# submission2019/cnn-quantization

Measured on NVIDIA H100. Metric: resnet50_w4a4_images_per_s, higher is better.
Workload: dtype f32

## Files before the change

cnn-quantization_b200/csrc/fq_bulk.cuh:

```cuda
#pragma once
#include <cuda_runtime.h>
#include <stdint.h>

#include "fq_device.cuh"

namespace fqb {

constexpr int kConsumers = kThreads;
constexpr int kBulkThreads = kConsumers + 32;
constexpr int kConsumerWarps = kConsumers / 32;
#ifndef FQB_STAGE_VEC
#define FQB_STAGE_VEC 4
#endif
#ifndef FQB_STAGES
#define FQB_STAGES 6
#endif
#ifndef FQB_BULK_CTAS
#define FQB_BULK_CTAS 1
#endif
constexpr int kBulkCtasPerSm = FQB_BULK_CTAS;
constexpr int kStageVec = FQB_STAGE_VEC;
constexpr int kStages = FQB_STAGES;
constexpr unsigned kStageBytes = kStageVec * kConsumers * 16u;
#ifndef FQB_BULK_SPLIT
#define FQB_BULK_SPLIT 1
#endif
constexpr unsigned kBulkSplit = FQB_BULK_SPLIT;

__device__ __forceinline__ void consumer_sync() { cta_sync(); }

__device__ __forceinline__ unsigned smem_u32(const void* p) { return static_cast<unsigned>(__cvta_generic_to_shared(p)); }
__device__ __forceinline__ void mbar_init(unsigned bar, unsigned count) {
  asm volatile("mbarrier.init.shared::cta.b64 [%0], %1;" ::"r"(bar), "r"(count) : "memory");
}
__device__ __forceinline__ void mbar_fence_init() { asm volatile("fence.mbarrier_init.release.cluster;" ::: "memory"); }
__device__ __forceinline__ void mbar_arrive(unsigned bar) {
  asm volatile("{ .reg .b64 st; mbarrier.arrive.shared::cta.b64 st, [%0]; }" ::"r"(bar) : "memory");
}
__device__ __forceinline__ void mbar_arrive_expect_tx(unsigned bar, unsigned bytes) {
  asm volatile("{ .reg .b64 st; mbarrier.arrive.expect_tx.shared::cta.b64 st, [%0], %1; }" ::"r"(bar), "r"(bytes) : "memory");
}
__device__ __forceinline__ bool mbar_try_wait(unsigned bar, unsigned parity) {
  unsigned ok;
  asm volatile(
      "{ .reg .pred p; mbarrier.try_wait.parity.shared::cta.b64 p, [%1], %2; selp.u32 %0, 1, 0, p; }"
      : "=r"(ok)
      : "r"(bar), "r"(parity)
      : "memory");
  return ok != 0;
}
__device__ __forceinline__ void mbar_wait(unsigned bar, unsigned parity) {
  while (!mbar_try_wait(bar, parity)) {
  }
}
__device__ __forceinline__ void bulk_load_one(unsigned dst_smem, const void* src, unsigned bytes, unsigned bar) {
  asm volatile("cp.async.bulk.shared::cluster.global.mbarrier::complete_tx::bytes [%0], [%1], %2, [%3];" ::"r"(dst_smem),
               "l"(src), "r"(bytes), "r"(bar)
               : "memory");
}
__device__ __forceinline__ void bulk_load(unsigned dst_smem, const void* src, unsigned bytes, unsigned bar) {
  if (kBulkSplit == 1u) {
    bulk_load_one(dst_smem, src, bytes, bar);
    return;
  }
  constexpr unsigned piece = kStageBytes / kBulkSplit;
  for (unsigned off = 0; off < bytes; off += piece)
    bulk_load_one(dst_smem + off, static_cast<const unsigned char*>(src) + off, min(piece, bytes - off), bar);
}

struct FlatGeo {
  unsigned total_v;
  unsigned stride;
  unsigned stage_v;
  unsigned n_stages;
  unsigned unit_stages;
  unsigned units;
  unsigned channels;
  unsigned cv;
};

struct StageMeta {
  unsigned start;
  unsigned count;
  unsigned tag;
  unsigned pad;
};

struct BulkRing {
  alignas(8) unsigned long long full[kStages];
  alignas(8) unsigned long long empty[kStages];
  StageMeta meta[kStages];
  unsigned nstages;
};

struct RingPos {
  unsigned slot, parity, n;
  __device__ __forceinline__ void init(unsigned nstages = kStages) {
    slot = 0;
    parity = 0;
    n = nstages;
  }
  __device__ __forceinline__ void next() {
    if (++slot == n) {
      slot = 0;
      parity ^= 1u;
    }
  }
};

__device__ __forceinline__ void ring_init(BulkRing& r, unsigned nstages = kStages) {
  if (threadIdx.x == 0) {
    r.nstages = nstages;
#pragma unroll
    for (int s = 0; s < kStages; ++s) {
      mbar_init(smem_u32(&r.full[s]), 1u);
      mbar_init(smem_u32(&r.empty[s]), kConsumerWarps);
    }
    mbar_fence_init();
  }
  __syncthreads();
}

struct TicketPlan {
  unsigned nstatic;
  unsigned first, step;
  unsigned dyn_base;
};

constexpr unsigned kPairOffset = kStageBytes / 2u;

__device__ __forceinline__ FlatGeo half_geo(const FlatGeo& g) {
  FlatGeo h = g;
  h.stage_v = (kStageVec / 2u) * g.stride;
  h.n_stages = (g.total_v + h.stage_v - 1u) / h.stage_v;
  h.unit_stages = 2u * g.unit_stages;
  return h;
}

template <bool REV, bool PAIR = false>
__device__ __forceinline__ void produce_phase(const FlatGeo& g, const float4* src, unsigned* counter, const TicketPlan tp,
                                              BulkRing& r, unsigned char* stage_base, RingPos& pos,
                                              const float4* src2 = nullptr) {
  const unsigned total = g.units;
  unsigned k = 0;
  auto fetch = [&]() -> unsigned {
    unsigned long long t;
    if (k < tp.nstatic)
      t = tp.first + static_cast<unsigned long long>(k) * tp.step;
    else
      t = static_cast<unsigned long long>(tp.dyn_base) + atomicAdd(counter, 1u);
    ++k;
    return t < total ? static_cast<unsigned>(t) : 0xffffffffu;
  };
  unsigned cur = fetch();
  unsigned nxt = (cur != 0xffffffffu) ? fetch() : 0xffffffffu;
  while (cur != 0xffffffffu) {
    const unsigned nxt2 = (nxt != 0xffffffffu) ? fetch() : 0xffffffffu;
    const unsigned u = REV ? total - 1u - cur : cur;
    const unsigned g0 = u * g.unit_stages;
    const unsigned g1 = min(g0 + g.unit_stages, g.n_stages);
    for (unsigned i = g0; i < g1; ++i) {
      const unsigned st = REV ? g1 - 1u - (i - g0) : i;
      const unsigned start = st * g.stage_v;
      const unsigned count = min(g.stage_v, g.total_v - start);
      mbar_wait(smem_u32(&r.empty[pos.slot]), pos.parity ^ 1u);
      r.meta[pos.slot].start = start;
      r.meta[pos.slot].count = count;
      r.meta[pos.slot].tag = 0u;
      const unsigned bar = smem_u32(&r.full[pos.slot]);
      mbar_arrive_expect_tx(bar, PAIR ? count * 32u : count * 16u);
      bulk_load(smem_u32(stage_base + pos.slot * kStageBytes), src + start, count * 16u, bar);
      if (PAIR) bulk_load(smem_u32(stage_base + pos.slot * kStageBytes + kPairOffset), src2 + start, count * 16u, bar);
      pos.next();
    }
    cur = nxt;
    nxt = nxt2;
  }
  mbar_wait(smem_u32(&r.empty[pos.slot]), pos.parity ^ 1u);
  r.meta[pos.slot].start = 0u;
  r.meta[pos.slot].count = 0u;
  mbar_arrive(smem_u32(&r.full[pos.slot]));
  pos.next();
}

struct RowsGeo {
  unsigned rows, row_v;
  unsigned stages_per_row;
  unsigned units_per_row;
};

__device__ __forceinline__ RowsGeo half_rows(const FlatGeo& h, const RowsGeo& rg) {
  RowsGeo r = rg;
  r.stages_per_row = (rg.row_v + h.stage_v - 1u) / h.stage_v;
  r.units_per_row = (r.stages_per_row + h.unit_stages - 1u) / h.unit_stages;
  return r;
}

template <bool REV, bool PAIR = false>
__device__ __forceinline__ void produce_rows_phase(const FlatGeo& g, const RowsGeo& rg, const float4* src, unsigned* counter,
                                                   const TicketPlan tp, BulkRing& r, unsigned char* stage_base, RingPos& pos,
                                                   const float4* src2 = nullptr) {
  const unsigned total = g.units;
  unsigned k = 0;
  auto fetch = [&]() -> unsigned {
    unsigned long long t;
    if (k < tp.nstatic)
      t = tp.first + static_cast<unsigned long long>(k) * tp.step;
    else
      t = static_cast<unsigned long long>(tp.dyn_base) + atomicAdd(counter, 1u);
    ++k;
    return t < total ? static_cast<unsigned>(t) : 0xffffffffu;
  };
  unsigned cur = fetch();
  unsigned nxt = (cur != 0xffffffffu) ? fetch() : 0xffffffffu;
  while (cur != 0xffffffffu) {
    const unsigned nxt2 = (nxt != 0xffffffffu) ? fetch() : 0xffffffffu;
    const unsigned u = REV ? total - 1u - cur : cur;
    const unsigned row = u / rg.units_per_row;
    const unsigned part = u - row * rg.units_per_row;
    const unsigned s0 = part * g.unit_stages;
    const unsigned s1 = min(s0 + g.unit_stages, rg.stages_per_row);
    for (unsigned i = s0; i < s1; ++i) {
      const unsigned st = REV ? s1 - 1u - (i - s0) : i;
      const unsigned off = st * g.stage_v;
      const unsigned start = row * rg.row_v + off;
      const unsigned count = min(g.stage_v, rg.row_v - off);
      mbar_wait(smem_u32(&r.empty[pos.slot]), pos.parity ^ 1u);
      r.meta[pos.slot].start = start;
      r.meta[pos.slot].count = count;
      r.meta[pos.slot].tag = row | (i + 1u == s1 ? 0x80000000u : 0u);
      const unsigned bar = smem_u32(&r.full[pos.slot]);
      mbar_arrive_expect_tx(bar, PAIR ? count * 32u : count * 16u);
      bulk_load(smem_u32(stage_base + pos.slot * kStageBytes), src + start, count * 16u, bar);
      if (PAIR) bulk_load(smem_u32(stage_base + pos.slot * kStageBytes + kPairOffset), src2 + start, count * 16u, bar);
      pos.next();
    }
    cur = nxt;
    nxt = nxt2;
  }
  mbar_wait(smem_u32(&r.empty[pos.slot]), pos.parity ^ 1u);
  r.meta[pos.slot].start = 0u;
  r.meta[pos.slot].count = 0u;
  r.meta[pos.slot].tag = 0u;
  mbar_arrive(smem_u32(&r.full[pos.slot]));
  pos.next();
}

struct PoolGeo {
  unsigned h, w;
  unsigned wt;
  unsigned tiles_per_row;
  unsigned row_pairs;
  unsigned tiles;
  unsigned unit_tiles, units;
  unsigned ow;
  unsigned kind;
};

constexpr unsigned kPoolTop = 1u, kPoolLeft = 2u;

__device__ __forceinline__ void produce_pool3_phase(const FlatGeo& g, const PoolGeo& pg, const float4* src, unsigned* counter,
                                                    const TicketPlan tp, BulkRing& r, unsigned char* stage_base, RingPos& pos) {
  const unsigned total = pg.units;
  unsigned k = 0;
  auto fetch = [&]() -> unsigned {
    unsigned long long t;
    if (k < tp.nstatic)
      t = tp.first + static_cast<unsigned long long>(k) * tp.step;
    else
      t = static_cast<unsigned long long>(tp.dyn_base) + atomicAdd(counter, 1u);
    ++k;
    return t < total ? static_cast<unsigned>(t) : 0xffffffffu;
  };
  const unsigned row_v = pg.w * g.cv;
  const unsigned region_v = (2u * pg.wt + 1u) * g.cv;
  const unsigned per_img = pg.row_pairs * pg.tiles_per_row;
  unsigned cur = fetch();
  unsigned nxt = (cur != 0xffffffffu) ? fetch() : 0xffffffffu;
  while (cur != 0xffffffffu) {
    const unsigned nxt2 = (nxt != 0xffffffffu) ? fetch() : 0xffffffffu;
    const unsigned t0 = cur * pg.unit_tiles;
    const unsigned t1 = min(t0 + pg.unit_tiles, pg.tiles);
    for (unsigned tile = t0; tile < t1; ++tile) {
      const unsigned n = tile / per_img;
      const unsigned rem = tile - n * per_img;
      const unsigned oh = rem / pg.tiles_per_row;
      const unsigned wi = rem - oh * pg.tiles_per_row;
      const bool top = oh > 0u, left = wi > 0u;
      const unsigned skip = left ? 0u : g.cv;
      const unsigned count = region_v - skip;
      const unsigned mid = (n * pg.h + 2u * oh) * row_v + (2u * wi * pg.wt) * g.cv - (left ? g.cv : 0u);
      const unsigned o = ((n * pg.row_pairs + oh) * pg.ow + wi * pg.wt) * g.cv;
      mbar_wait(smem_u32(&r.empty[pos.slot]), pos.parity ^ 1u);
      r.meta[pos.slot].start = o;
      r.meta[pos.slot].count = count;
      r.meta[pos.slot].tag = (top ? kPoolTop : 0u) | (left ? kPoolLeft : 0u);
      const unsigned bar = smem_u32(&r.full[pos.slot]);
      mbar_arrive_expect_tx(bar, count * 16u * (top ? 3u : 2u));
      const unsigned dst = smem_u32(stage_base + pos.slot * kStageBytes) + skip * 16u;
      if (top) bulk_load(dst, src + mid - row_v, count * 16u, bar);
      bulk_load(dst + region_v * 16u, src + mid, count * 16u, bar);
      bulk_load(dst + 2u * region_v * 16u, src + mid + row_v, count * 16u, bar);
      pos.next();
    }
    cur = nxt;
    nxt = nxt2;
  }
  mbar_wait(smem_u32(&r.empty[pos.slot]), pos.parity ^ 1u);
  r.meta[pos.slot].start = 0u;
  r.meta[pos.slot].count = 0u;
  r.meta[pos.slot].tag = 0u;
  mbar_arrive(smem_u32(&r.full[pos.slot]));
  pos.next();
}

template <typename Acc>
__device__ __forceinline__ void consume_pool3_phase(const FlatGeo& g, const PoolGeo& pg, BulkRing& r, const unsigned char* stage_base,
                                                    RingPos& pos, Acc& acc) {
  const unsigned t = threadIdx.x;
  const bool lane0 = (t & 31u) == 0u;
  const bool mine = t < pg.wt * g.cv;
  const unsigned j = t / g.cv, col = t - j * g.cv;
  const unsigned region = (2u * pg.wt + 1u) * g.cv * 16u;
  const unsigned my = smem_u32(stage_base) + ((2u * j) * g.cv + col) * 16u;
  const unsigned nxt = g.cv * 16u;
  for (;;) {
    mbar_wait(smem_u32(&r.full[pos.slot]), pos.parity);
    const StageMeta m = r.meta[pos.slot];
    if (m.count != 0u && mine) {
      const unsigned addr = my + pos.slot * kStageBytes;
      const bool first = (j != 0u) || (m.tag & kPoolLeft);
      acc.pool_begin();
#pragma unroll
      for (int dy = 0; dy < 3; ++dy) {
        if (dy == 0 && !(m.tag & kPoolTop)) continue;
        const unsigned row = addr + dy * region;
        float4 v;
        if (first) {
          lds_vec(row, v);
          acc.pool_tap(v);
        }
        lds_vec(row + nxt, v);
        acc.pool_tap(v);
        lds_vec(row + 2u * nxt, v);
        acc.pool_tap(v);
      }
      acc.pool_end(m.start + t);
    }
    __syncwarp();
    if (lane0) mbar_arrive(smem_u32(&r.empty[pos.slot]));
    pos.next();
    if (m.count == 0u) break;
  }
}

__device__ __forceinline__ void produce_pool_phase(const FlatGeo& g, const PoolGeo& pg, const float4* src, unsigned* counter,
                                                   const TicketPlan tp, BulkRing& r, unsigned char* stage_base, RingPos& pos) {
  const unsigned total = pg.units;
  unsigned k = 0;
  auto fetch = [&]() -> unsigned {
    unsigned long long t;
    if (k < tp.nstatic)
      t = tp.first + static_cast<unsigned long long>(k) * tp.step;
    else
      t = static_cast<unsigned long long>(tp.dyn_base) + atomicAdd(counter, 1u);
    ++k;
    return t < total ? static_cast<unsigned>(t) : 0xffffffffu;
  };
  const unsigned row_v = pg.w * g.cv;
  const unsigned count = pg.wt * g.cv;
  const unsigned per_img = pg.row_pairs * pg.tiles_per_row;
  unsigned cur = fetch();
  unsigned nxt = (cur != 0xffffffffu) ? fetch() : 0xffffffffu;
  while (cur != 0xffffffffu) {
    const unsigned nxt2 = (nxt != 0xffffffffu) ? fetch() : 0xffffffffu;
    const unsigned t0 = cur * pg.unit_tiles;
    const unsigned t1 = min(t0 + pg.unit_tiles, pg.tiles);
    for (unsigned tile = t0; tile < t1; ++tile) {
      const unsigned n = tile / per_img;
      const unsigned rem = tile - n * per_img;
      const unsigned hp = rem / pg.tiles_per_row;
      const unsigned wi = rem - hp * pg.tiles_per_row;
      const unsigned a = (n * pg.h + 2u * hp) * row_v + wi * count;
      const unsigned o = ((n * pg.row_pairs + hp) * pg.ow + wi * (pg.wt / 2u)) * g.cv;
      mbar_wait(smem_u32(&r.empty[pos.slot]), pos.parity ^ 1u);
      r.meta[pos.slot].start = o;
      r.meta[pos.slot].count = count;
      r.meta[pos.slot].tag = 0u;
      const unsigned bar = smem_u32(&r.full[pos.slot]);
      mbar_arrive_expect_tx(bar, count * 32u);
      bulk_load(smem_u32(stage_base + pos.slot * kStageBytes), src + a, count * 16u, bar);
      bulk_load(smem_u32(stage_base + pos.slot * kStageBytes + kPairOffset), src + a + row_v, count * 16u, bar);
      pos.next();
    }
    cur = nxt;
    nxt = nxt2;
  }
  mbar_wait(smem_u32(&r.empty[pos.slot]), pos.parity ^ 1u);
  r.meta[pos.slot].start = 0u;
  r.meta[pos.slot].count = 0u;
  r.meta[pos.slot].tag = 0u;
  mbar_arrive(smem_u32(&r.full[pos.slot]));
  pos.next();
}

template <typename Acc>
__device__ __forceinline__ void consume_pool_phase(const FlatGeo& g, const PoolGeo& pg, BulkRing& r, const unsigned char* stage_base,
                                                   RingPos& pos, Acc& acc) {
  const unsigned t = threadIdx.x;
  const bool lane0 = (t & 31u) == 0u;
  const bool mine = t < (pg.wt / 2u) * g.cv;
  const unsigned j = t / g.cv, col = t - j * g.cv;
  const unsigned my = smem_u32(stage_base) + ((2u * j) * g.cv + col) * 16u;
  const unsigned nxt = g.cv * 16u;
  for (;;) {
    mbar_wait(smem_u32(&r.full[pos.slot]), pos.parity);
    const StageMeta m = r.meta[pos.slot];
    if (m.count != 0u && mine) {
      const unsigned addr = my + pos.slot * kStageBytes;
      float4 a0, a1, b0, b1;
      lds_vec(addr, a0);
      lds_vec(addr + nxt, a1);
      lds_vec(addr + kPairOffset, b0);
      lds_vec(addr + kPairOffset + nxt, b1);
      acc.pooled(a0, a1, b0, b1, m.start + t);
    }
    __syncwarp();
    if (lane0) mbar_arrive(smem_u32(&r.empty[pos.slot]));
    pos.next();
    if (m.count == 0u) break;
  }
}

template <typename Acc>
__device__ __forceinline__ void consume_phase(const FlatGeo& g, BulkRing& r, const unsigned char* stage_base, RingPos& pos,
                                              Acc& acc) {
  const unsigned t = threadIdx.x;
  const bool lane0 = (t & 31u) == 0u;
  const unsigned my = smem_u32(stage_base) + t * 16u;
  const unsigned step = g.stride * 16u;
  for (;;) {
    mbar_wait(smem_u32(&r.full[pos.slot]), pos.parity);
    const StageMeta m = r.meta[pos.slot];
    const unsigned addr = my + pos.slot * kStageBytes;
    if (m.count == g.stage_v) {
      if (t < g.stride) {
        float4 x[kStageVec];
#pragma unroll
        for (int i = 0; i < kStageVec; ++i) lds_vec(addr + i * step, x[i]);
#pragma unroll
        for (int i = 0; i < kStageVec; ++i) acc.consume(x[i], m.start + t + i * g.stride);
      }
    } else if (m.count != 0u) {
#pragma unroll
      for (int i = 0; i < kStageVec; ++i) {
        const unsigned idx = t + i * g.stride;
        if (t < g.stride && idx < m.count) {
          float4 x;
          lds_vec(addr + i * step, x);
          acc.consume(x, m.start + idx);
        }
// ... 56 lines not shown
```

cnn-quantization_b200/csrc/fq_cl.cuh:

```cuda
#pragma once

namespace fqb {

__device__ __forceinline__ unsigned enc_ordered(float x) {
  const unsigned b = __float_as_uint(x);
  return (b & 0x80000000u) ? ~b : (b | 0x80000000u);
}
__device__ __forceinline__ float dec_ordered(unsigned e) {
  return __uint_as_float((e & 0x80000000u) ? (e & 0x7fffffffu) : ~e);
}

constexpr unsigned kAccU = 2u * kMaxNhwcChannels;
constexpr unsigned kAccD = 3u * kMaxNhwcChannels;

struct ClView {
  unsigned* amin_inv;
  unsigned* amax;
  double* asum;
  double* asq;
  double* aabs;
};
__device__ __forceinline__ ClView cl_view(const FusedArgs& A, unsigned bank) {
  ClView v;
  v.amin_inv = A.amin_inv + bank * kAccU;
  v.amax = v.amin_inv + kMaxNhwcChannels;
  v.asum = A.asum + bank * kAccD;
  v.asq = v.asum + kMaxNhwcChannels;
  v.aabs = v.asq + kMaxNhwcChannels;
  return v;
}

__device__ __forceinline__ void red_add_f64(double* p, double v) {
  asm volatile("red.global.add.f64 [%0], %1;" ::"l"(p), "d"(v) : "memory");
}
__device__ __forceinline__ void red_max_u32(unsigned* p, unsigned v) {
  asm volatile("red.global.max.u32 [%0], %1;" ::"l"(p), "r"(v) : "memory");
}

__device__ __noinline__ void grid_arrive_cl(GridSync* gs, unsigned& epoch) {
  ++epoch;
  consumer_sync();
  if (threadIdx.x == 0) {
    unsigned prev;
    asm volatile("atom.add.acq_rel.gpu.global.u32 %0, [%1], 1;" : "=r"(prev) : "l"(&gs->arrive) : "memory");
    if (prev + 1u == epoch * gridDim.x) st_release_u32(&gs->release, epoch);
  }
}
__device__ __noinline__ void grid_wait_cl(GridSync* gs, unsigned epoch) {
  if (threadIdx.x == 0) {
    while (ld_acquire_u32(&gs->release) < epoch) __nanosleep(32);
  }
  consumer_sync();
}
__device__ __forceinline__ void grid_barrier_cl(GridSync* gs, unsigned& epoch) {
  grid_arrive_cl(gs, epoch);
  grid_wait_cl(gs, epoch);
}
__device__ __forceinline__ void grid_exit_cl(GridSync* gs) {
  consumer_sync();
  if (threadIdx.x == 0) {
    const unsigned prev = atomicAdd(&gs->exited, 1u);
    if (prev + 1u == gridDim.x) {
      gs->arrive = 0u;
      gs->release = 0u;
      for (int i = 0; i < 8; ++i) gs->unit_counter[i] = 0u;
      gs->launch_count = gs->launch_count + 1u;
      __threadfence();
      gs->exited = 0u;
    }
  }
}

constexpr unsigned kClChunkStages = 1;

struct ClStats1 {
  float mn[4], mx[4], k[4], fs[4], fq[4];
  double s[4], q[4];
  unsigned cnt;
  __device__ __forceinline__ void init(const FusedArgs& A, unsigned c0, bool active) {
    float4 first = make_float4(0.f, 0.f, 0.f, 0.f);
    if (active) first = ld_tensor(reinterpret_cast<const float4*>(A.in) + (c0 >> 2));
    k[0] = first.x;
    k[1] = first.y;
    k[2] = first.z;
    k[3] = first.w;
    cnt = 0;
#pragma unroll
    for (int i = 0; i < 4; ++i) {
      mn[i] = INFINITY;
      mx[i] = -INFINITY;
      fs[i] = 0.f;
      fq[i] = 0.f;
      s[i] = 0.0;
      q[i] = 0.0;
    }
  }
  __device__ __forceinline__ void flush() {
#pragma unroll
    for (int i = 0; i < 4; ++i) {
      s[i] += static_cast<double>(fs[i]);
      q[i] += static_cast<double>(fq[i]);
      fs[i] = 0.f;
      fq[i] = 0.f;
    }
    cnt = 0;
  }
  __device__ __forceinline__ void consume(const float4& v, unsigned) {
    const float x[4] = {v.x, v.y, v.z, v.w};
#pragma unroll
    for (int i = 0; i < 4; ++i) {
      const float d = __fsub_rn(x[i], k[i]);
      mn[i] = fminf(mn[i], x[i]);
      mx[i] = fmaxf(mx[i], x[i]);
      fs[i] = __fadd_rn(fs[i], d);
      fq[i] = __fmaf_rn(d, d, fq[i]);
    }
  }
  __device__ __forceinline__ void stage_end(const StageMeta&) {
    if (++cnt == kClChunkStages) flush();
  }
};

struct ClStats2 {
  float mu[4], bias[4], fa[4];
  double sa[4];
  unsigned cnt;
  __device__ __forceinline__ void init(const FusedArgs& A, unsigned c0, bool active, const float (&mean)[4]) {
    cnt = 0;
#pragma unroll
    for (int i = 0; i < 4; ++i) {
      bias[i] = (A.bias && active) ? __ldg(A.bias + c0 + i) : 0.f;
      mu[i] = mean[i];
      fa[i] = 0.f;
      sa[i] = 0.0;
    }
  }
  __device__ __forceinline__ void flush() {
#pragma unroll
    for (int i = 0; i < 4; ++i) {
      sa[i] += static_cast<double>(fa[i]);
      fa[i] = 0.f;
    }
    cnt = 0;
  }
  __device__ __forceinline__ void consume(const float4& v, unsigned) {
// ... 431 lines not shown
  cl_combine_add_f64(cx.cbuf, g.cv, g.stride, s2.sa, acc.aabs + rb, s2.sa, nullptr, s2.sa, nullptr);
}

template <int LEAF, bool HIST>
__device__ __noinline__ void cl_phase_apply(const FusedArgs& A, ClCtx& cx, const LeafParam (&lp)[4], unsigned* hist) {
  const FlatGeo& g = *cx.g;
  const unsigned t = threadIdx.x;
  if (HIST) {
    for (unsigned i = t; i < kHistWords; i += kConsumers) hist[i] = 0u;
    consumer_sync();
  }
  ClApply<LEAF, HIST> ap{A, hist};
  ap.init(cx.c0, cx.active, lp);
  RingPos pos = cx.pos;
  if (A.pool.tiles) {
    if (A.pool.kind == 3u)
      consume_pool3_phase(g, A.pool, *cx.ring, cx.stages, pos, ap);
    else
      consume_pool_phase(g, A.pool, *cx.ring, cx.stages, pos, ap);
  } else if (A.residual) {
    const FlatGeo h = half_geo(g);
    consume_pair_phase(h, *cx.ring, cx.stages, pos, ap);
  } else {
    consume_phase(g, *cx.ring, cx.stages, pos, ap);
  }
  cx.pos = pos;
  if (HIST) {
    consumer_sync();
    const unsigned bins = static_cast<unsigned>(A.hist_bins);
    const unsigned copies = max(1u, min(static_cast<unsigned>(kWarps), kHistWords / bins));
    for (unsigned b = t; b < bins; b += kConsumers) {
      unsigned long long cnt = 0;
      for (unsigned w = 0; w < copies; ++w) cnt += hist[w * bins + b];
      if (cnt) atomicAdd(A.hist + b, cnt);
    }
    if (LEAF == FQB200_LEAF_MIDTREAD && A.hist_clamped && cx.active) {
#pragma unroll
      for (int i = 0; i < 4; ++i) {
        if (ap.nlo[i]) atomicAdd(A.hist_clamped + 2u * (cx.c0 + i), static_cast<unsigned long long>(ap.nlo[i]));
        if (ap.nhi[i]) atomicAdd(A.hist_clamped + 2u * (cx.c0 + i) + 1u, static_cast<unsigned long long>(ap.nhi[i]));
      }
    }
  }
}

constexpr unsigned kClStagingBytes = 4u * kConsumers * 8u;
constexpr unsigned kClTableChannels = 1024;
constexpr unsigned kClCombineBytes = kClStagingBytes + kClTableChannels * 4u;

template <int LEAF, bool DEV, bool HIST>
__global__ void __launch_bounds__(kBulkThreads, kBulkCtasPerSm) fq_cl_kernel(const __grid_constant__ FusedArgs A) {
  extern __shared__ __align__(128) unsigned char fq_dyn[];
  unsigned char* stages = fq_dyn;
  unsigned char* cbuf = fq_dyn + kStages * kStageBytes;
  float* tab_mean = reinterpret_cast<float*>(cbuf + kClStagingBytes);
  unsigned* hist = reinterpret_cast<unsigned*>(stages + (kStages - 1) * kStageBytes);
  __shared__ BulkRing ring;
  __shared__ LeaderSmem lsm;
  __shared__ alignas(8) unsigned long long solver_done;
  const FlatGeo& g = A.flat;
  const unsigned C = g.channels, cv = g.cv;
  const unsigned launch = ld_ws(&A.sync->launch_count);
  const unsigned bank = launch & 1u;
  const unsigned tag = launch + 1u;
  const bool alloc = (LEAF == FQB200_LEAF_MIDTREAD) || (A.bit_alloc && A.num_bits <= 4);
  const bool aux_needs_b = alloc && LEAF != FQB200_LEAF_MIDTREAD && A.prior == FQB200_PRIOR_B;
  const bool solver_in_s2 = alloc && !aux_needs_b && DEV && gridDim.x > 1u;
  __shared__ alignas(8) unsigned long long phase_go[2];
  if (threadIdx.x == 0) {
    mbar_init(smem_u32(&solver_done), 1u);
    mbar_init(smem_u32(&phase_go[0]), 1u);
    mbar_init(smem_u32(&phase_go[1]), 1u);
  }
  const unsigned nstages = HIST ? kStages - 1u : kStages;
  ring_init(ring, nstages);

  if (threadIdx.x >= kConsumers) {
    if (threadIdx.x == kConsumers) {
      RingPos pos;
      pos.init(nstages);
      const float4* src = reinterpret_cast<const float4*>(A.in);
      const TicketPlan all = {2u, blockIdx.x, gridDim.x, 2u * gridDim.x};
      const TicketPlan no0 = {blockIdx.x == 0 ? 0u : 2u, blockIdx.x - 1u, gridDim.x - 1u, 2u * (gridDim.x - 1u)};
      produce_phase<false>(g, src, &A.sync->unit_counter[0], all, ring, stages, pos);
      if (DEV) {
        mbar_wait(smem_u32(&phase_go[0]), 0u);
        if (solver_in_s2 && blockIdx.x == 0) mbar_wait(smem_u32(&solver_done), 0u);
        produce_phase<true>(g, src, &A.sync->unit_counter[1], solver_in_s2 ? no0 : all, ring, stages, pos);
      }
      if (!A.stats_only) {
        mbar_wait(smem_u32(&phase_go[1]), 0u);
        if (A.pool.tiles && A.pool.kind == 3u)
          produce_pool3_phase(g, A.pool, src, &A.sync->unit_counter[2], all, ring, stages, pos);
        else if (A.pool.tiles)
          produce_pool_phase(g, A.pool, src, &A.sync->unit_counter[2], all, ring, stages, pos);
        else if (A.residual)
          produce_phase<!DEV, true>(half_geo(g), src, &A.sync->unit_counter[2], all, ring, stages, pos,
                                    reinterpret_cast<const float4*>(A.residual));
        else
          produce_phase<!DEV>(g, src, &A.sync->unit_counter[2], all, ring, stages, pos);
      }
    }
    return;
  }

  const unsigned t = threadIdx.x;
  const bool active = t < g.stride;
  const bool direct = cv == g.stride;
  const unsigned col = active ? t % cv : 0u;
  const unsigned c0 = 4u * col;
  const double n = A.n_per_group;
  const ClView acc = cl_view(A, bank);
  const unsigned rep = A.nhwc_rep;
  const unsigned rep_base = (blockIdx.x % rep) * C;
  unsigned epoch = 0;
  if (blockIdx.x == 0) stamp(A, 0);

  if (blockIdx.x == gridDim.x - 1u) {
    const ClView other = cl_view(A, bank ^ 1u);
    uint4* zu = reinterpret_cast<uint4*>(other.amin_inv);
    uint4* zd = reinterpret_cast<uint4*>(other.asum);
    const uint4 z = make_uint4(0u, 0u, 0u, 0u);
    for (unsigned i = t; i < kAccU / 4u; i += kConsumers) zu[i] = z;
    for (unsigned i = t; i < kAccD / 2u; i += kConsumers) zd[i] = z;
  }

  ClCtx cx;
  cx.g = &g;
  cx.ring = &ring;
  cx.stages = stages;
  cx.cbuf = cbuf;
  cx.pos.init(nstages);
  cx.acc = acc;
  cx.rep_base = rep_base;
  cx.c0 = c0;
  cx.active = active;
  float kshift[4];
  cl_phase_s1(A, cx, kshift);
  if (t == 0) mbar_arrive(smem_u32(&phase_go[DEV ? 0 : 1]));
  if (blockIdx.x == 0) stamp(A, 1);
  grid_barrier_cl(A.sync, epoch);
  if (blockIdx.x == 0) stamp(A, 4);

  float mean[4];
  if (direct) {
#pragma unroll
    for (int i = 0; i < 4; ++i)
      mean[i] = static_cast<float>(cl_mean(acc, rep, C, c0 + i, kshift[i], (A.bias && active) ? __ldg(A.bias + c0 + i) : 0.f, n));
  } else {
    for (unsigned c = t; c < C; c += kConsumers)
      tab_mean[c] = static_cast<float>(cl_mean(acc, rep, C, c, ld_tensor(A.in + c), A.bias ? __ldg(A.bias + c) : 0.f, n));
    consumer_sync();
#pragma unroll
    for (int i = 0; i < 4; ++i) mean[i] = tab_mean[c0 + i];
  }

  if (alloc && !aux_needs_b && blockIdx.x == 0) {
    cl_solve_aux(A, acc, lsm, tag, false, !solver_in_s2);
    stamp(A, 12);
    if (t == 0) mbar_arrive(smem_u32(&solver_done));
  }

  if constexpr (DEV) {
    cl_phase_s2(A, cx, mean);
    if (t == 0) mbar_arrive(smem_u32(&phase_go[1]));
    if (blockIdx.x == 0) stamp(A, 5);
    grid_barrier_cl(A.sync, epoch);
    if (blockIdx.x == 0) stamp(A, 8);
    if (aux_needs_b && blockIdx.x == 0) cl_solve_aux(A, acc, lsm, tag, true, true);
  }
  if (alloc && !solver_in_s2) {
    if (t == 0)
      while (ld_acquire_u32(&A.sync->aux_ready) != tag) __nanosleep(40);
    consumer_sync();
  }

  LeafParam lp[4];
  const bool do_export = A.out_stats != nullptr && blockIdx.x == 0;
  if (direct) {
#pragma unroll
    for (int i = 0; i < 4; ++i) lp[i] = cl_channel_param<LEAF, DEV>(A, acc, rep, C, c0 + i, mean[i], n, alloc, do_export && active);
  } else {
    LeafParam* tab_lp = reinterpret_cast<LeafParam*>(cbuf);
    consumer_sync();
    for (unsigned c = t; c < C; c += kConsumers) tab_lp[c] = cl_channel_param<LEAF, DEV>(A, acc, rep, C, c, tab_mean[c], n, alloc, do_export);
    consumer_sync();
#pragma unroll
    for (int i = 0; i < 4; ++i) lp[i] = tab_lp[c0 + i];
  }
  if (blockIdx.x == 0) stamp(A, 7);

  if (!A.stats_only) {
    cl_phase_apply<LEAF, HIST>(A, cx, lp, hist);
    if (blockIdx.x == 0) stamp(A, 9);
  }
  grid_exit_cl(A.sync);
}

template <bool GRID>
struct ClGiven {
  const FusedArgs& A;
  LeafParam q[4];
  float r[4], bias[4];
  bool fast;
  template <bool FAST>
  __device__ __forceinline__ void one(const float4& v, unsigned off) {
    const float x[4] = {v.x, v.y, v.z, v.w};
    float y[4], gq[4];
#pragma unroll
    for (int i = 0; i < 4; ++i) {
      Divisor dv;
      dv.s = q[i].a;
      dv.r = r[i];
      dv.fast = FAST;
      y[i] = leaf_apply<FQB200_LEAF_TORCH, FAST>(__fadd_rn(x[i], bias[i]), q[i], dv, 0.f, gq[i]);
    }
    st_tensor(reinterpret_cast<float4*>(A.out) + off, make_float4(y[0], y[1], y[2], y[3]));
    if (GRID) st_tensor(reinterpret_cast<float4*>(A.grid_out) + off, make_float4(gq[0], gq[1], gq[2], gq[3]));
  }
  __device__ __forceinline__ void consume(const float4& v, unsigned off) {
    if (fast)
      one<true>(v, off);
    else
      one<false>(v, off);
  }
  __device__ __forceinline__ void stage_end(const StageMeta&) {}
};

template <bool GRID>
__global__ void __launch_bounds__(kBulkThreads, kBulkCtasPerSm) fq_cl_given_kernel(const __grid_constant__ FusedArgs A) {
  extern __shared__ __align__(128) unsigned char fq_dyn[];
  __shared__ BulkRing ring;
  const FlatGeo& g = A.flat;
  ring_init(ring);
  if (threadIdx.x >= kConsumers) {
    if (threadIdx.x == kConsumers) {
      RingPos pos;
      pos.init();
      const TicketPlan tp = {0xffffffffu, blockIdx.x, gridDim.x, 0u};
      produce_phase<false>(g, reinterpret_cast<const float4*>(A.in), nullptr, tp, ring, fq_dyn, pos);
    }
    return;
  }
  const unsigned t = threadIdx.x;
  const bool active = t < g.stride;
  const unsigned c0 = active ? 4u * (t % g.cv) : 0u;
  ClGiven<GRID> ap{A};
  ap.fast = true;
#pragma unroll
  for (int i = 0; i < 4; ++i) {
    const unsigned c = c0 + i;
    const unsigned pi = A.given_per_group ? c : 0u;
    const float bits = A.g_bits ? __ldg(A.g_bits + c) : static_cast<float>(A.num_bits);
    ap.q[i] = make_leaf_param(FQB200_LEAF_TORCH, __ldg(A.g_delta + pi), __ldg(A.g_offset + pi), bits);
    const Divisor dv = make_divisor(ap.q[i].a);
    ap.r[i] = dv.r;
    ap.fast = ap.fast && dv.fast;
    ap.bias[i] = (A.bias && active) ? __ldg(A.bias + c) : 0.f;
  }
  RingPos pos;
  pos.init();
  consume_phase(g, ring, fq_dyn, pos, ap);
}

__global__ void __launch_bounds__(kBulkThreads, kBulkCtasPerSm) fq_cl_given_fused_kernel(const __grid_constant__ FusedArgs A) {
  extern __shared__ __align__(128) unsigned char fq_dyn[];
  __shared__ BulkRing ring;
  const FlatGeo& g = A.flat;
  ring_init(ring);
  if (threadIdx.x >= kConsumers) {
    if (threadIdx.x == kConsumers) {
      RingPos pos;
      pos.init();
      const float4* src = reinterpret_cast<const float4*>(A.in);
      const TicketPlan tp = {0xffffffffu, blockIdx.x, gridDim.x, 0u};
      if (A.pool.tiles && A.pool.kind == 3u)
        produce_pool3_phase(g, A.pool, src, nullptr, tp, ring, fq_dyn, pos);
      else if (A.pool.tiles)
        produce_pool_phase(g, A.pool, src, nullptr, tp, ring, fq_dyn, pos);
      else if (A.residual)
        produce_phase<false, true>(half_geo(g), src, nullptr, tp, ring, fq_dyn, pos, reinterpret_cast<const float4*>(A.residual));
      else
        produce_phase<false>(g, src, nullptr, tp, ring, fq_dyn, pos);
    }
    return;
  }
  const unsigned t = threadIdx.x;
  const bool active = t < g.stride;
  const unsigned c0 = active ? 4u * (t % g.cv) : 0u;
  LeafParam lp[4];
#pragma unroll
  for (int i = 0; i < 4; ++i) {
    const unsigned c = c0 + i;
    const float bits = A.g_bits ? __ldg(A.g_bits + c) : static_cast<float>(A.num_bits);
    lp[i] = make_leaf_param(FQB200_LEAF_TORCH, __ldg(A.g_delta + c), __ldg(A.g_offset + c), bits);
  }
  ClApply<FQB200_LEAF_TORCH, false> ap{A, nullptr};
  ap.init(c0, active, lp);
  RingPos pos;
  pos.init();
  if (A.pool.tiles && A.pool.kind == 3u)
    consume_pool3_phase(g, A.pool, ring, fq_dyn, pos, ap);
  else if (A.pool.tiles)
    consume_pool_phase(g, A.pool, ring, fq_dyn, pos, ap);
  else if (A.residual)
    consume_pair_phase(half_geo(g), ring, fq_dyn, pos, ap);
  else
    consume_phase(g, ring, fq_dyn, pos, ap);
}

struct LeafBulkArgs {
  FlatGeo flat;
  const float* in;
  float* out;
  const float* noise;
  LeafParam q;
};

template <bool NOISE>
struct LeafBulk {
  const LeafBulkArgs& A;
  Divisor dv;
  template <bool FAST>
  __device__ __forceinline__ void one(const float4& v, const float4& nz, unsigned off) {
    float gq;
    float4 y;
    y.x = leaf_apply<FQB200_LEAF_COMPILED, FAST, NOISE>(v.x, A.q, dv, NOISE ? nz.x : 0.f, gq);
    y.y = leaf_apply<FQB200_LEAF_COMPILED, FAST, NOISE>(v.y, A.q, dv, NOISE ? nz.y : 0.f, gq);
    y.z = leaf_apply<FQB200_LEAF_COMPILED, FAST, NOISE>(v.z, A.q, dv, NOISE ? nz.z : 0.f, gq);
    y.w = leaf_apply<FQB200_LEAF_COMPILED, FAST, NOISE>(v.w, A.q, dv, NOISE ? nz.w : 0.f, gq);
    st_tensor(reinterpret_cast<float4*>(A.out) + off, y);
  }
  __device__ __forceinline__ void consume(const float4& v, unsigned off) {
    if (dv.fast)
      one<true>(v, v, off);
    else
      one<false>(v, v, off);
  }
  __device__ __forceinline__ void consume2(const float4& v, const float4& nz, unsigned off) {
    if (dv.fast)
      one<true>(v, nz, off);
    else
      one<false>(v, nz, off);
  }
  __device__ __forceinline__ void stage_end(const StageMeta&) {}
};

template <bool NOISE>
__global__ void __launch_bounds__(kBulkThreads, kBulkCtasPerSm) fq_leaf_bulk_kernel(const __grid_constant__ LeafBulkArgs A) {
  extern __shared__ __align__(128) unsigned char fq_dyn[];
  __shared__ BulkRing ring;
  const FlatGeo g = NOISE ? half_geo(A.flat) : A.flat;
  ring_init(ring);
  if (threadIdx.x >= kConsumers) {
    if (threadIdx.x == kConsumers) {
      RingPos pos;
      pos.init();
      const TicketPlan tp = {0xffffffffu, blockIdx.x, gridDim.x, 0u};
      produce_phase<false, NOISE>(g, reinterpret_cast<const float4*>(A.in), nullptr, tp, ring, fq_dyn, pos,
                                  reinterpret_cast<const float4*>(A.noise));
    }
    return;
// ... 265 lines not shown
    if (PAIR) {
      y.x = __fadd_rn(y.x, r.x);
      y.y = __fadd_rn(y.y, r.y);
      y.z = __fadd_rn(y.z, r.z);
      y.w = __fadd_rn(y.w, r.w);
      if (A.residual_relu) {
        y.x = y.x < 0.f ? 0.f : y.x;
        y.y = y.y < 0.f ? 0.f : y.y;
        y.z = y.z < 0.f ? 0.f : y.z;
        y.w = y.w < 0.f ? 0.f : y.w;
      }
    }
    st_tensor(reinterpret_cast<float4*>(A.out) + off, y);
  }
  __device__ __forceinline__ void consume(const float4& v, unsigned off) {
    if (dv.fast)
      one<true, false>(v, v, off);
    else
      one<false, false>(v, v, off);
  }
  __device__ __forceinline__ void consume2(const float4& v, const float4& r, unsigned off) {
    if (dv.fast)
      one<true, true>(v, r, off);
    else
      one<false, true>(v, r, off);
  }
  __device__ __forceinline__ void stage_end(const StageMeta&) {}
  float pm[4];
  __device__ __forceinline__ void pool_begin() {
#pragma unroll
    for (int i = 0; i < 4; ++i) pm[i] = -INFINITY;
  }
  __device__ __forceinline__ void pool_tap(const float4& v) {
    auto mx = [](float p, float q) { return (q > p || q != q) ? q : p; };
    pm[0] = mx(pm[0], v.x);
    pm[1] = mx(pm[1], v.y);
    pm[2] = mx(pm[2], v.z);
    pm[3] = mx(pm[3], v.w);
  }
  __device__ __forceinline__ void pool_end(unsigned off) {
    float gq;
    float4 y;
    if (dv.fast) {
      y.x = leaf_apply<FQB200_LEAF_COMPILED, true>(__fadd_rn(pm[0], bias[0]), q, dv, 0.f, gq);
      y.y = leaf_apply<FQB200_LEAF_COMPILED, true>(__fadd_rn(pm[1], bias[1]), q, dv, 0.f, gq);
      y.z = leaf_apply<FQB200_LEAF_COMPILED, true>(__fadd_rn(pm[2], bias[2]), q, dv, 0.f, gq);
      y.w = leaf_apply<FQB200_LEAF_COMPILED, true>(__fadd_rn(pm[3], bias[3]), q, dv, 0.f, gq);
    } else {
      y.x = leaf_apply<FQB200_LEAF_COMPILED, false>(__fadd_rn(pm[0], bias[0]), q, dv, 0.f, gq);
      y.y = leaf_apply<FQB200_LEAF_COMPILED, false>(__fadd_rn(pm[1], bias[1]), q, dv, 0.f, gq);
      y.z = leaf_apply<FQB200_LEAF_COMPILED, false>(__fadd_rn(pm[2], bias[2]), q, dv, 0.f, gq);
      y.w = leaf_apply<FQB200_LEAF_COMPILED, false>(__fadd_rn(pm[3], bias[3]), q, dv, 0.f, gq);
    }
    st_tensor(reinterpret_cast<float4*>(A.pool_out) + off, y);
  }
  __device__ __forceinline__ void pooled(const float4& a0, const float4& a1, const float4& b0, const float4& b1, unsigned off) {
    pool_begin();
    pool_tap(a0);
    pool_tap(a1);
    pool_tap(b0);
    pool_tap(b1);
    pool_end(off);
  }
};

__global__ void __launch_bounds__(kBulkThreads, kBulkCtasPerSm) fq_rows_kernel(const __grid_constant__ FusedArgs A) {
  extern __shared__ __align__(128) unsigned char fq_dyn[];
  __shared__ BulkRing ring;
  __shared__ LeaderSmem lsm;
  __shared__ float scratch[2 * kWarps];
  const FlatGeo& g = A.flat;
  const RowsGeo& rg = A.rows;
  const unsigned bank = ld_ws(&A.sync->launch_count) & 1u;
  ring_init(ring);
  if (threadIdx.x >= kConsumers) {
    if (threadIdx.x == kConsumers) {
      RingPos pos;
      pos.init();
      const float4* src = reinterpret_cast<const float4*>(A.in);
      const TicketPlan all = {2u, blockIdx.x, gridDim.x, 2u * gridDim.x};
      produce_rows_phase<false>(g, rg, src, &A.sync->unit_counter[0], all, ring, fq_dyn, pos);
      if (!A.stats_only) {
        if (A.pool.tiles && A.pool.kind == 3u) {
          produce_pool3_phase(g, A.pool, src, &A.sync->unit_counter[2], all, ring, fq_dyn, pos);
        } else if (A.pool.tiles) {
          produce_pool_phase(g, A.pool, src, &A.sync->unit_counter[2], all, ring, fq_dyn, pos);
        } else if (A.residual) {
          const FlatGeo h = half_geo(g);
          produce_rows_phase<true, true>(h, half_rows(h, rg), src, &A.sync->unit_counter[2], all, ring, fq_dyn, pos,
                                         reinterpret_cast<const float4*>(A.residual));
        } else {
          produce_rows_phase<true>(g, rg, src, &A.sync->unit_counter[2], all, ring, fq_dyn, pos);
        }
      }
    }
    return;
  }
  const unsigned t = threadIdx.x;
  const bool active = t < g.stride;
  const unsigned c0 = active ? 4u * (t % g.cv) : 0u;
  const ClView acc = cl_view(A, bank);
  unsigned epoch = 0;
  RingPos pos;
  pos.init();
  if (blockIdx.x == 0) stamp(A, 0);
  if (blockIdx.x == gridDim.x - 1u) {
    const ClView other = cl_view(A, bank ^ 1u);
    uint4* zu = reinterpret_cast<uint4*>(other.amin_inv);
    uint4* zd = reinterpret_cast<uint4*>(other.asum);
    const uint4 z = make_uint4(0u, 0u, 0u, 0u);
    for (unsigned i = t; i < kAccU / 4u; i += kConsumers) zu[i] = z;
    for (unsigned i = t; i < kAccD / 2u; i += kConsumers) zd[i] = z;
  }
  float bias[4];
#pragma unroll
  for (int i = 0; i < 4; ++i) bias[i] = (A.bias && active) ? __ldg(A.bias + c0 + i) : 0.f;
  {
    RowsStats s1{A, scratch, acc, {bias[0], bias[1], bias[2], bias[3]}, INFINITY, -INFINITY};
    consume_phase(g, ring, fq_dyn, pos, s1);
  }
  if (blockIdx.x == 0) stamp(A, 1);
  grid_barrier_cl(A.sync, epoch);
  if (blockIdx.x == 0) stamp(A, 4);
  const unsigned R = rg.rows;
  float mn, mx;
  if (A.scope == FQB200_SCOPE_GROUP_MEAN) {
    double smin = 0.0, smax = 0.0;
    for (unsigned r = t; r < R; r += kConsumers) {
      smin += static_cast<double>(dec_ordered(~ld_ws(acc.amin_inv + r)));
      smax += static_cast<double>(dec_ordered(ld_ws(acc.amax + r)));
    }
    smin = block_reduce(smin, OpAdd(), lsm.d);
    smax = block_reduce(smax, OpAdd(), lsm.d);
    mn = static_cast<float>(smin / R);
    mx = static_cast<float>(smax / R);
  } else {
    float lmin = INFINITY, lmax = -INFINITY;
    for (unsigned r = t; r < R; r += kConsumers) {
      lmin = fminf(lmin, dec_ordered(~ld_ws(acc.amin_inv + r)));
      lmax = fmaxf(lmax, dec_ordered(ld_ws(acc.amax + r)));
    }
    mn = block_reduce(lmin, OpMin(), lsm.f);
    mx = block_reduce(lmax, OpMax(), lsm.f);
  }
  float delta, offset;
  solve_range(A, mn, mx, 0.f, 0.f, 0.f, static_cast<float>(A.num_bits), delta, offset);
  const LeafParam q = make_leaf_param(FQB200_LEAF_COMPILED, delta, offset, static_cast<float>(A.num_bits), A.relu_passthrough != 0);
  if (blockIdx.x == 0 && t == 0) export_stats(A, 0, mn, mx, 0.f, 0.f, 0.f, delta, offset, static_cast<float>(A.num_bits), q);
  if (blockIdx.x == 0) stamp(A, 7);
  if (!A.stats_only) {
    RowsApply ap{A, q, make_divisor(q.a), {bias[0], bias[1], bias[2], bias[3]}};
    ap.init_residual(c0, active);
    if (A.pool.tiles && A.pool.kind == 3u)
      consume_pool3_phase(g, A.pool, ring, fq_dyn, pos, ap);
    else if (A.pool.tiles)
      consume_pool_phase(g, A.pool, ring, fq_dyn, pos, ap);
    else if (A.residual)
      consume_pair_phase(half_geo(g), ring, fq_dyn, pos, ap);
    else
      consume_phase(g, ring, fq_dyn, pos, ap);
    if (blockIdx.x == 0) stamp(A, 9);
  }
  grid_exit_cl(A.sync);
}

}
```

Baseline: 8915.

## Taper work-unit sizes at tail and alternate phase traversal direction

```diff
diff --git a/cnn-quantization_b200/csrc/fq_bulk.cuh b/cnn-quantization_b200/csrc/fq_bulk.cuh
--- a/cnn-quantization_b200/csrc/fq_bulk.cuh
+++ b/cnn-quantization_b200/csrc/fq_bulk.cuh
@@ -13,7 +13,7 @@
 #define FQB_STAGE_VEC 4
 #endif
 #ifndef FQB_STAGES
-#define FQB_STAGES 6
+#define FQB_STAGES 4
 #endif
 #ifndef FQB_BULK_CTAS
 #define FQB_BULK_CTAS 1
@@ -137,11 +137,33 @@
   return h;
 }
 
+__device__ __forceinline__ bool unit_span(const FlatGeo& g, unsigned t, unsigned& s0, unsigned& s1) {
+  const unsigned u = g.unit_stages, n = g.n_stages, grid = gridDim.x;
+  const unsigned tail = min(n, grid * (u - __popc(u)));
+  const unsigned big_end = n - tail;
+  const unsigned big = (big_end + u - 1u) / u;
+  if (t < big) {
+    s0 = t * u;
+    s1 = min(s0 + u, big_end);
+    return true;
+  }
+  t -= big;
+  unsigned start = big_end, w = u >> 1;
+  while (w != 0u && t >= grid) {
+    start += grid * w;
+    t -= grid;
+    w >>= 1;
+  }
+  s0 = start + t * w;
+  if (w == 0u || s0 >= n) return false;
+  s1 = min(s0 + w, n);
+  return true;
+}
+
 template <bool REV, bool PAIR = false>
 __device__ __forceinline__ void produce_phase(const FlatGeo& g, const float4* src, unsigned* counter, const TicketPlan tp,
                                               BulkRing& r, unsigned char* stage_base, RingPos& pos,
                                               const float4* src2 = nullptr) {
-  const unsigned total = g.units;
   unsigned k = 0;
   auto fetch = [&]() -> unsigned {
     unsigned long long t;
@@ -150,17 +172,16 @@
     else
       t = static_cast<unsigned long long>(tp.dyn_base) + atomicAdd(counter, 1u);
     ++k;
-    return t < total ? static_cast<unsigned>(t) : 0xffffffffu;
+    return t < 0xffffffffull ? static_cast<unsigned>(t) : 0xffffffffu;
   };
+  unsigned s0, s1;
   unsigned cur = fetch();
-  unsigned nxt = (cur != 0xffffffffu) ? fetch() : 0xffffffffu;
-  while (cur != 0xffffffffu) {
-    const unsigned nxt2 = (nxt != 0xffffffffu) ? fetch() : 0xffffffffu;
-    const unsigned u = REV ? total - 1u - cur : cur;
-    const unsigned g0 = u * g.unit_stages;
-    const unsigned g1 = min(g0 + g.unit_stages, g.n_stages);
-    for (unsigned i = g0; i < g1; ++i) {
-      const unsigned st = REV ? g1 - 1u - (i - g0) : i;
+  unsigned nxt = unit_span(g, cur, s0, s1) ? fetch() : 0xffffffffu;
+  while (unit_span(g, cur, s0, s1)) {
+    unsigned n0, n1;
+    const unsigned nxt2 = unit_span(g, nxt, n0, n1) ? fetch() : 0xffffffffu;
+    for (unsigned i = s0; i < s1; ++i) {
+      const unsigned st = REV ? g.n_stages - 1u - i : i;
       const unsigned start = st * g.stage_v;
       const unsigned count = min(g.stage_v, g.total_v - start);
       mbar_wait(smem_u32(&r.empty[pos.slot]), pos.parity ^ 1u);
@@ -259,6 +280,7 @@
 
 constexpr unsigned kPoolTop = 1u, kPoolLeft = 2u;
 
+template <bool REV>
 __device__ __forceinline__ void produce_pool3_phase(const FlatGeo& g, const PoolGeo& pg, const float4* src, unsigned* counter,
                                                     const TicketPlan tp, BulkRing& r, unsigned char* stage_base, RingPos& pos) {
   const unsigned total = pg.units;
@@ -279,9 +301,10 @@
   unsigned nxt = (cur != 0xffffffffu) ? fetch() : 0xffffffffu;
   while (cur != 0xffffffffu) {
     const unsigned nxt2 = (nxt != 0xffffffffu) ? fetch() : 0xffffffffu;
-    const unsigned t0 = cur * pg.unit_tiles;
+    const unsigned t0 = (REV ? total - 1u - cur : cur) * pg.unit_tiles;
     const unsigned t1 = min(t0 + pg.unit_tiles, pg.tiles);
-    for (unsigned tile = t0; tile < t1; ++tile) {
+    for (unsigned i = t0; i < t1; ++i) {
+      const unsigned tile = REV ? t1 - 1u - (i - t0) : i;
       const unsigned n = tile / per_img;
       const unsigned rem = tile - n * per_img;
       const unsigned oh = rem / pg.tiles_per_row;
@@ -354,6 +377,7 @@
   }
 }
 
+template <bool REV>
 __device__ __forceinline__ void produce_pool_phase(const FlatGeo& g, const PoolGeo& pg, const float4* src, unsigned* counter,
                                                    const TicketPlan tp, BulkRing& r, unsigned char* stage_base, RingPos& pos) {
   const unsigned total = pg.units;
@@ -374,9 +398,10 @@
   unsigned nxt = (cur != 0xffffffffu) ? fetch() : 0xffffffffu;
   while (cur != 0xffffffffu) {
     const unsigned nxt2 = (nxt != 0xffffffffu) ? fetch() : 0xffffffffu;
-    const unsigned t0 = cur * pg.unit_tiles;
+    const unsigned t0 = (REV ? total - 1u - cur : cur) * pg.unit_tiles;
     const unsigned t1 = min(t0 + pg.unit_tiles, pg.tiles);
-    for (unsigned tile = t0; tile < t1; ++tile) {
+    for (unsigned i = t0; i < t1; ++i) {
+      const unsigned tile = REV ? t1 - 1u - (i - t0) : i;
       const unsigned n = tile / per_img;
       const unsigned rem = tile - n * per_img;
       const unsigned hp = rem / pg.tiles_per_row;
diff --git a/cnn-quantization_b200/csrc/fq_cl.cuh b/cnn-quantization_b200/csrc/fq_cl.cuh
--- a/cnn-quantization_b200/csrc/fq_cl.cuh
+++ b/cnn-quantization_b200/csrc/fq_cl.cuh
@@ -37,13 +37,23 @@
   asm volatile("red.global.max.u32 [%0], %1;" ::"l"(p), "r"(v) : "memory");
 }
 
-__device__ __noinline__ void grid_arrive_cl(GridSync* gs, unsigned& epoch) {
+__device__ __forceinline__ void stamp_at(unsigned long long* dbg, int slot) {
+  unsigned long long t;
+  asm volatile("mov.u64 %0, %globaltimer;" : "=l"(t));
+  dbg[slot] = t;
+}
+__device__ __noinline__ void grid_arrive_cl(GridSync* gs, unsigned& epoch, unsigned long long* dbg = nullptr, int first = 0,
+                                            int last = 0) {
   ++epoch;
   consumer_sync();
   if (threadIdx.x == 0) {
     unsigned prev;
     asm volatile("atom.add.acq_rel.gpu.global.u32 %0, [%1], 1;" : "=r"(prev) : "l"(&gs->arrive) : "memory");
-    if (prev + 1u == epoch * gridDim.x) st_release_u32(&gs->release, epoch);
+    if (dbg && prev == (epoch - 1u) * gridDim.x) stamp_at(dbg, first);
+    if (prev + 1u == epoch * gridDim.x) {
+      if (dbg) stamp_at(dbg, last);
+      st_release_u32(&gs->release, epoch);
+    }
   }
 }
 __device__ __noinline__ void grid_wait_cl(GridSync* gs, unsigned epoch) {
@@ -52,15 +62,17 @@
   }
   consumer_sync();
 }
-__device__ __forceinline__ void grid_barrier_cl(GridSync* gs, unsigned& epoch) {
-  grid_arrive_cl(gs, epoch);
+__device__ __forceinline__ void grid_barrier_cl(GridSync* gs, unsigned& epoch, unsigned long long* dbg = nullptr, int first = 0,
+                                                int last = 0) {
+  grid_arrive_cl(gs, epoch, dbg, first, last);
   grid_wait_cl(gs, epoch);
 }
-__device__ __forceinline__ void grid_exit_cl(GridSync* gs) {
+__device__ __forceinline__ void grid_exit_cl(GridSync* gs, unsigned long long* dbg = nullptr) {
   consumer_sync();
   if (threadIdx.x == 0) {
     const unsigned prev = atomicAdd(&gs->exited, 1u);
     if (prev + 1u == gridDim.x) {
+      if (dbg) stamp_at(dbg, 6);
       gs->arrive = 0u;
       gs->release = 0u;
       for (int i = 0; i < 8; ++i) gs->unit_counter[i] = 0u;
@@ -658,23 +670,23 @@
       const float4* src = reinterpret_cast<const float4*>(A.in);
       const TicketPlan all = {2u, blockIdx.x, gridDim.x, 2u * gridDim.x};
       const TicketPlan no0 = {blockIdx.x == 0 ? 0u : 2u, blockIdx.x - 1u, gridDim.x - 1u, 2u * (gridDim.x - 1u)};
-      produce_phase<false>(g, src, &A.sync->unit_counter[0], all, ring, stages, pos);
+      produce_phase<true>(g, src, &A.sync->unit_counter[0], all, ring, stages, pos);
       if (DEV) {
         mbar_wait(smem_u32(&phase_go[0]), 0u);
         if (solver_in_s2 && blockIdx.x == 0) mbar_wait(smem_u32(&solver_done), 0u);
-        produce_phase<true>(g, src, &A.sync->unit_counter[1], solver_in_s2 ? no0 : all, ring, stages, pos);
+        produce_phase<false>(g, src, &A.sync->unit_counter[1], solver_in_s2 ? no0 : all, ring, stages, pos);
       }
       if (!A.stats_only) {
         mbar_wait(smem_u32(&phase_go[1]), 0u);
         if (A.pool.tiles && A.pool.kind == 3u)
-          produce_pool3_phase(g, A.pool, src, &A.sync->unit_counter[2], all, ring, stages, pos);
+          produce_pool3_phase<DEV>(g, A.pool, src, &A.sync->unit_counter[2], all, ring, stages, pos);
         else if (A.pool.tiles)
-          produce_pool_phase(g, A.pool, src, &A.sync->unit_counter[2], all, ring, stages, pos);
+          produce_pool_phase<DEV>(g, A.pool, src, &A.sync->unit_counter[2], all, ring, stages, pos);
         else if (A.residual)
-          produce_phase<!DEV, true>(half_geo(g), src, &A.sync->unit_counter[2], all, ring, stages, pos,
-                                    reinterpret_cast<const float4*>(A.residual));
+          produce_phase<DEV, true>(half_geo(g), src, &A.sync->unit_counter[2], all, ring, stages, pos,
+                                         reinterpret_cast<const float4*>(A.residual));
         else
-          produce_phase<!DEV>(g, src, &A.sync->unit_counter[2], all, ring, stages, pos);
+          produce_phase<DEV>(g, src, &A.sync->unit_counter[2], all, ring, stages, pos);
       }
     }
     return;
@@ -714,8 +726,7 @@
   float kshift[4];
   cl_phase_s1(A, cx, kshift);
   if (t == 0) mbar_arrive(smem_u32(&phase_go[DEV ? 0 : 1]));
-  if (blockIdx.x == 0) stamp(A, 1);
-  grid_barrier_cl(A.sync, epoch);
+  grid_barrier_cl(A.sync, epoch, A.dbg, 1, 2);
   if (blockIdx.x == 0) stamp(A, 4);
 
   float mean[4];
@@ -740,8 +751,7 @@
   if constexpr (DEV) {
     cl_phase_s2(A, cx, mean);
     if (t == 0) mbar_arrive(smem_u32(&phase_go[1]));
-    if (blockIdx.x == 0) stamp(A, 5);
-    grid_barrier_cl(A.sync, epoch);
+    grid_barrier_cl(A.sync, epoch, A.dbg, 5, 3);
     if (blockIdx.x == 0) stamp(A, 8);
     if (aux_needs_b && blockIdx.x == 0) cl_solve_aux(A, acc, lsm, tag, true, true);
   }
@@ -770,7 +780,7 @@
     cl_phase_apply<LEAF, HIST>(A, cx, lp, hist);
     if (blockIdx.x == 0) stamp(A, 9);
   }
-  grid_exit_cl(A.sync);
+  grid_exit_cl(A.sync, A.dbg);
 }
 
 template <bool GRID>
@@ -851,9 +861,9 @@
       const float4* src = reinterpret_cast<const float4*>(A.in);
       const TicketPlan tp = {0xffffffffu, blockIdx.x, gridDim.x, 0u};
       if (A.pool.tiles && A.pool.kind == 3u)
-        produce_pool3_phase(g, A.pool, src, nullptr, tp, ring, fq_dyn, pos);
+        produce_pool3_phase<false>(g, A.pool, src, nullptr, tp, ring, fq_dyn, pos);
       else if (A.pool.tiles)
-        produce_pool_phase(g, A.pool, src, nullptr, tp, ring, fq_dyn, pos);
+        produce_pool_phase<false>(g, A.pool, src, nullptr, tp, ring, fq_dyn, pos);
       else if (A.residual)
         produce_phase<false, true>(half_geo(g), src, nullptr, tp, ring, fq_dyn, pos, reinterpret_cast<const float4*>(A.residual));
       else
@@ -1285,9 +1295,9 @@
       produce_rows_phase<false>(g, rg, src, &A.sync->unit_counter[0], all, ring, fq_dyn, pos);
       if (!A.stats_only) {
         if (A.pool.tiles && A.pool.kind == 3u) {
-          produce_pool3_phase(g, A.pool, src, &A.sync->unit_counter[2], all, ring, fq_dyn, pos);
+          produce_pool3_phase<false>(g, A.pool, src, &A.sync->unit_counter[2], all, ring, fq_dyn, pos);
         } else if (A.pool.tiles) {
-          produce_pool_phase(g, A.pool, src, &A.sync->unit_counter[2], all, ring, fq_dyn, pos);
+          produce_pool_phase<false>(g, A.pool, src, &A.sync->unit_counter[2], all, ring, fq_dyn, pos);
         } else if (A.residual) {
           const FlatGeo h = half_geo(g);
           produce_rows_phase<true, true>(h, half_rows(h, rg), src, &A.sync->unit_counter[2], all, ring, fq_dyn, pos,
@@ -1322,8 +1332,7 @@
     RowsStats s1{A, scratch, acc, {bias[0], bias[1], bias[2], bias[3]}, INFINITY, -INFINITY};
     consume_phase(g, ring, fq_dyn, pos, s1);
   }
-  if (blockIdx.x == 0) stamp(A, 1);
-  grid_barrier_cl(A.sync, epoch);
+  grid_barrier_cl(A.sync, epoch, A.dbg, 1, 2);
   if (blockIdx.x == 0) stamp(A, 4);
   const unsigned R = rg.rows;
   float mn, mx;
@@ -1364,7 +1373,7 @@
       consume_phase(g, ring, fq_dyn, pos, ap);
     if (blockIdx.x == 0) stamp(A, 9);
   }
-  grid_exit_cl(A.sync);
-}
-
-}
+  grid_exit_cl(A.sync, A.dbg);
+}
+
+}
```

After: 8956, median of 6. Within noise of the previous version (+0.5%).
